# cristicbz/rust-doom

Measured on NVIDIA H100. Metric: frames/sec at 1920x1080 (palette-index bit-exact), higher is better.
Workload: dtype u8

## Files before the change

### rust-doom_b200/csrc/b2d_kernels.cu

```cuda
#include <type_traits>

#include "b2d_kernels.cuh"

namespace b2d {

namespace {

constexpr unsigned kFull = 0xFFFFFFFFu;

constexpr int kMaskWords = 128;
constexpr int kStackDepth = 128;

constexpr uint32_t kVisBit = 1u << 25, kSolidBit = 1u << 24;
__device__ __forceinline__ uint32_t pack_range(int lo, int hi, uint32_t bits) {
    return (uint32_t)lo | ((uint32_t)hi << 12) | bits;
}
__device__ __forceinline__ int range_lo(uint32_t r) { return (int)(r & 0xFFFu); }
__device__ __forceinline__ int range_hi(uint32_t r) { return (int)((r >> 12) & 0xFFFu); }

__device__ __forceinline__ uint32_t word_bits(int w, int lo, int hi) {
    int a = max(lo, w * 32), b = min(hi, w * 32 + 31);
    if (a > b) return 0u;
    uint32_t m = 0xFFFFFFFFu >> (31 - (b - w * 32));
    return m & (0xFFFFFFFFu << (a - w * 32));
// ... 360 lines not shown

constexpr int kBatch = 8;

template <bool kRgba, int kW>
__device__ __forceinline__ void store_batch(const RasterCtx &c, uint8_t *p8, uint32_t *p32, const uint32_t (&v)[kBatch],
                                            int y, int ya, int yb, bool full) {
    const int Wc = kW ? kW : c.W;
    if (full) {
#pragma unroll
        for (int k = 0; k < kBatch; k++) put_px<kRgba>(c, p8 + (size_t)k * Wc, kRgba ? p32 + (size_t)k * Wc : nullptr, true, v[k]);
    } else {
        const uint32_t m = row_mask(y, ya, yb, kBatch);
#pragma unroll
        for (int k = 0; k < kBatch; k++)
            put_px<kRgba>(c, p8 + (size_t)k * Wc, kRgba ? p32 + (size_t)k * Wc : nullptr, (m >> k) & 1u, v[k]);
    }
}

template <bool kRgba, int kW>
__device__ __forceinline__ void fill_void_warp(const RasterCtx &c, int ya, int yb) {
    bool act = ya < yb;
    int y0 = __reduce_min_sync(kFull, act ? ya : 0x7FFFFFFF);
    int y1 = __reduce_max_sync(kFull, act ? yb : 0);
    if (y0 >= y1) return;
    const int Wc = kW ? kW : c.W;
    uint8_t *p8 = c.fb + (size_t)y0 * Wc;
    uint32_t *p32 = kRgba ? c.rgba + (size_t)y0 * Wc : nullptr;
#pragma unroll 1
    for (int y = y0; y < y1; y++, p8 += Wc, p32 += Wc) put_px<kRgba>(c, p8, p32, y >= ya && y < yb, 0u);
}

template <bool kRgba, int kW>
__device__ __forceinline__ void draw_sky_warp(const RasterCtx &c, int ya, int yb) {
    const DeviceScene &sc = *c.sc;
    if (sc.sky_tex < 0) { fill_void_warp<kRgba, kW>(c, ya, yb); return; }
    const TexRec T = sc.tex[sc.sky_tex];
    const bool inter = tex_interleaved(T);
    const uint8_t *px = sc.lit_texels + T.texel_off + (inter ? 4u * c.skycol : c.skycol);
    const uint32_t w4 = 4u * T.w;
    bool act = ya < yb;
    int y0 = __reduce_min_sync(kFull, act ? ya : 0x7FFFFFFF);
    int y1 = __reduce_max_sync(kFull, act ? yb : 0);
    if (y0 >= y1) return;
    const int Wc = kW ? kW : c.W;
    uint8_t *p8 = c.fb + (size_t)y0 * Wc;
    uint32_t *p32 = kRgba ? c.rgba + (size_t)y0 * Wc : nullptr;
#pragma unroll 2
    for (int y = y0; y < y1; y++, p8 += Wc, p32 += Wc) {
        const uint32_t r = sc.skyrow[y];
        put_px<kRgba>(c, p8, p32, y >= ya && y < yb, __ldg(px + (inter ? (r >> 2) * w4 + (r & 3u) : r * T.w)));
    }
}

template <bool kRgba, int kW, bool kFixed = false>
__device__ __forceinline__ void draw_plane_warp(const RasterCtx &c, const FrameConst &fc, const View &vw,
                                                int ya, int yb, int32_t h, int32_t flat, int lightb,
                                                bool visible) {
    const DeviceScene &sc = *c.sc;
    if (!__any_sync(kFull, ya < yb)) return;
    if (!visible) { fill_void_warp<kRgba, kW>(c, ya, yb); return; }
    if (flat == kFlatSky) { draw_sky_warp<kRgba, kW>(c, ya, yb); return; }
    if (flat < 0 || flat >= sc.nflats) { fill_void_warp<kRgba, kW>(c, ya, yb); return; }
    const uint8_t *lit_flats = sc.lit_flats;
    int fixed_row = -1;
    if constexpr (kFixed) {
        lit_flats = c.fix.row == 32 ? c.fix.flats : lit_flats;
        fixed_row = c.fix.row == 32 ? 0 : c.fix.row;
    }
    const uint64_t px_hi = reinterpret_cast<uint64_t>(lit_flats) & 0xFFFFFFFF00000000ull;
    const uint32_t habs = plane_habs(h, fc.pose.z);
    bool act = ya < yb;
    int y0 = __reduce_min_sync(kFull, act ? ya : 0x7FFFFFFF);
    int y1 = __reduce_max_sync(kFull, act ? yb : 0);
    const int full_lo = __reduce_max_sync(kFull, act ? ya : 0x7FFFFFFF);
    const int full_hi = __reduce_min_sync(kFull, act ? yb : 0);
    const int Wc = kW ? kW : c.W;
    uint8_t *p8 = c.fb + (size_t)y0 * Wc;
    uint32_t *p32 = kRgba ? c.rgba + (size_t)y0 * Wc : nullptr;
    const uint32_t bu = (uint32_t)fc.pose.x << 10, bv = (uint32_t)fc.pose.y << 10;
    const uint32_t ax = (uint32_t)c.dir.ax, ay = (uint32_t)c.dir.ay;
    for (int yc = y0; yc < y1; yc += 32) {
        int yy = yc + c.lane;
        if (yy < y1) {
            const PlaneRow pr = plane_row(habs, sc.yslope[yy]);
            c.rowz[c.lane] = make_uint2(pr.z8q, (sc.lit_flat_stride >> 6) * (uint32_t)(kFixed && fixed_row >= 0 ? fixed_row : light_row(lightb, pr.z8)) + 64u * (uint32_t)flat);
        }
        __syncwarp();
        const int rows = min(32, y1 - yc);
        int j = 0;
        for (; j + kBatch <= rows; j += kBatch, p8 += (size_t)kBatch * Wc, p32 += (size_t)kBatch * Wc) {
            uint32_t v[kBatch];
#pragma unroll
            for (int k = 0; k < kBatch; k++) {
                const uint2 rz = c.rowz[j + k];
                v[k] = __ldg(reinterpret_cast<const uint8_t *>(px_hi | flat_offset(rz.y, bu + rz.x * ax, bv + rz.x * ay)));
            }
            const int y = yc + j;
            store_batch<kRgba, kW>(c, p8, p32, v, y, ya, yb, y >= full_lo && y + kBatch <= full_hi);
        }
        for (; j < rows; j++, p8 += Wc, p32 += Wc) {
            const uint2 rz = c.rowz[j];
            const int y = yc + j;
            put_px<kRgba>(c, p8, p32, y >= ya && y < yb,
                          __ldg(reinterpret_cast<const uint8_t *>(px_hi | flat_offset(rz.y, bu + rz.x * ax, bv + rz.x * ay))));
        }
        __syncwarp();
    }
}

template <bool kRgba, int kW, int R>
__device__ __forceinline__ void wall_fast_loop(const RasterCtx &c, const uint8_t *plq, uint32_t w4, uint32_t nq, uint32_t q,
                                               uint32_t acc, uint32_t ts29, int y0, int y1, int ya, int yb,
                                               int full_lo, int full_hi) {
    const int Wc = kW ? kW : c.W;
    uint8_t *p8 = c.fb + (size_t)y0 * Wc;
    uint32_t *p32 = kRgba ? c.rgba + (size_t)y0 * Wc : nullptr;
    asm("" : "+l"(plq));
#pragma unroll 1
    for (int y = y0; y < y1; y += R, p8 += (size_t)R * Wc, p32 += (size_t)R * Wc) {
        const uint32_t q1 = q + 1u == nq ? 0u : q + 1u;
        const uint32_t w0 = __ldg(reinterpret_cast<const uint32_t *>(plq + (size_t)q * w4));
        const uint32_t w1 = __ldg(reinterpret_cast<const uint32_t *>(plq + (size_t)q1 * w4));
        if (y >= full_lo && y + R <= full_hi) {
#pragma unroll
            for (int k = 0; k < R; k++) {
                uint32_t v = pick_byte(w0, w1, wall_sel(acc, ts29, (uint32_t)k));
                if (kRgba) v &= 0xFFu;
                put_px<kRgba>(c, p8 + (size_t)k * Wc, kRgba ? p32 + (size_t)k * Wc : nullptr, true, v);
            }
        } else {
            const uint32_t m = row_mask(y, ya, yb, R);
#pragma unroll
            for (int k = 0; k < R; k++) {
                uint32_t v = pick_byte(w0, w1, wall_sel(acc, ts29, (uint32_t)k));
                if (kRgba) v &= 0xFFu;
                put_px<kRgba>(c, p8 + (size_t)k * Wc, kRgba ? p32 + (size_t)k * Wc : nullptr, (m >> k) & 1u, v);
            }
        }
        wall_advance(acc, q, ts29, (uint32_t)R, nq);
    }
}

template <bool kRgba, int kW, bool kFixed = false>
__device__ __forceinline__ void draw_wall_warp(const RasterCtx &c, const FrameConst &fc, int ya, int yb,
                                               int32_t tex, int32_t tA, int32_t hA, int32_t ucol,
                                               int32_t iscale, int row) {
    const DeviceScene &sc = *c.sc;
    if (!__any_sync(kFull, ya < yb)) return;
    if (tex < 0 || tex >= sc.ntex) { fill_void_warp<kRgba, kW>(c, ya, yb); return; }
    const TexRec T = sc.tex[tex];
    bool act = ya < yb;
    const uint32_t col = (uint32_t)floormod32(ucol, (int32_t)T.w);
    const uint8_t *pl = sc.lit_texels + (size_t)row * sc.lit_texel_stride + T.texel_off;
    if constexpr (kFixed) {
        if (row == 32) pl = c.fix.texels + T.texel_off;
    }
    const uint32_t tstep = (uint32_t)(iscale >> 4);
    int y0 = __reduce_min_sync(kFull, act ? ya : 0x7FFFFFFF);
    int y1 = __reduce_max_sync(kFull, act ? yb : 0);
    const int full_lo = __reduce_max_sync(kFull, act ? ya : 0x7FFFFFFF);
    const int full_hi = __reduce_min_sync(kFull, act ? yb : 0);
    uint32_t t = (uint32_t)wall_tbase(tA, hA, fc.pose.z, c.H, iscale) + (uint32_t)y0 * tstep;
    const int Wc = kW ? kW : c.W;
    uint8_t *p8 = c.fb + (size_t)y0 * Wc;
    uint32_t *p32 = kRgba ? c.rgba + (size_t)y0 * Wc : nullptr;
    if (tex_interleaved(T) && T.h >= 8u) {
        const uint32_t ts = act ? tstep : 0u;
        const bool f16 = __all_sync(kFull, ts <= kWallFast16);
        if (f16 || __all_sync(kFull, ts <= kWallFast8)) {
            const uint32_t tt = act ? t : 0u;
            const uint32_t r0 = wall_row((int32_t)tt, T.h, T.hmagic, T.hbias);
            const uint8_t *plq = pl + 4u * col;
            if (f16) wall_fast_loop<kRgba, kW, 16>(c, plq, 4u * T.w, T.h >> 2, r0 >> 2, wall_acc29(tt, r0), ts << 13, y0, y1, ya, yb, full_lo, full_hi);
            else wall_fast_loop<kRgba, kW, 8>(c, plq, 4u * T.w, T.h >> 2, r0 >> 2, wall_acc29(tt, r0), ts << 13, y0, y1, ya, yb, full_lo, full_hi);
            return;
        }
    }
    if (tex_interleaved(T)) {
        const uint32_t colb = 4u * col, w4 = 4u * T.w;
        for (int y = y0; y < y1; y += kBatch, p8 += (size_t)kBatch * Wc, p32 += (size_t)kBatch * Wc, t += (uint32_t)kBatch * tstep) {
            const uint32_t r0 = wall_row((int32_t)t, T.h, T.hmagic, T.hbias);
            const uint32_t acc = wall_acc(t, r0);
            const uint32_t b7 = (acc + 7u * tstep) >> 16;
            uint32_t v[kBatch];
            if (__all_sync(kFull, b7 < 8u)) {
                const uint32_t q0 = r0 >> 2, q1 = next_quad(q0, T.h);
                const uint32_t w0 = __ldg(reinterpret_cast<const uint32_t *>(pl + (q0 * w4 + colb)));
                const uint32_t w1 = __ldg(reinterpret_cast<const uint32_t *>(pl + (q1 * w4 + colb)));
#pragma unroll
                for (int k = 0; k < kBatch; k++) {
                    v[k] = pick_byte(w0, w1, (acc + (uint32_t)k * tstep) >> 16);
                    if (kRgba) v[k] &= 0xFFu;
                }
            } else {
                const uint32_t t4 = t + 4u * tstep;
                const uint32_t r4 = wall_row((int32_t)t4, T.h, T.hmagic, T.hbias);
                const uint32_t acc4 = wall_acc(t4, r4);
                if (__all_sync(kFull, ((acc + 3u * tstep) >> 16) < 8u && ((acc4 + 3u * tstep) >> 16) < 8u)) {
                    const uint32_t q0 = r0 >> 2, q4 = r4 >> 2;
                    const uint32_t a0 = __ldg(reinterpret_cast<const uint32_t *>(pl + (q0 * w4 + colb)));
                    const uint32_t a1 = __ldg(reinterpret_cast<const uint32_t *>(pl + (next_quad(q0, T.h) * w4 + colb)));
                    const uint32_t b0 = __ldg(reinterpret_cast<const uint32_t *>(pl + (q4 * w4 + colb)));
                    const uint32_t b1 = __ldg(reinterpret_cast<const uint32_t *>(pl + (next_quad(q4, T.h) * w4 + colb)));
#pragma unroll
                    for (int k = 0; k < 4; k++) {
                        v[k] = pick_byte(a0, a1, (acc + (uint32_t)k * tstep) >> 16);
                        v[k + 4] = pick_byte(b0, b1, (acc4 + (uint32_t)k * tstep) >> 16);
                        if (kRgba) { v[k] &= 0xFFu; v[k + 4] &= 0xFFu; }
                    }
                } else {
#pragma unroll
                    for (int k = 0; k < kBatch; k++) {
                        const uint32_t rk = wall_row((int32_t)(t + (uint32_t)k * tstep), T.h, T.hmagic, T.hbias);
                        v[k] = __ldg(pl + ((rk >> 2) * w4 + colb + (rk & 3u)));
                    }
                }
            }
            store_batch<kRgba, kW>(c, p8, p32, v, y, ya, yb, y >= full_lo && y + kBatch <= full_hi);
        }
    } else {
        const uint8_t *px = pl + col;
#pragma unroll 1
        for (int y = y0; y < y1; y++, p8 += Wc, p32 += Wc, t += tstep)
            put_px<kRgba>(c, p8, p32, y >= ya && y < yb, __ldg(px + wall_row((int32_t)t, T.h, T.hmagic, T.hbias) * T.w));
    }
}

__device__ __forceinline__ uint32_t *masked_entry(const DeviceScene &sc, const uint32_t *chunks, int e) {
    return sc.masked_list + ((size_t)chunks[e / kMaskedChunk] * kMaskedChunk + (size_t)(e % kMaskedChunk)) * 33u;
}
__device__ __forceinline__ uint32_t *masked_push(const DeviceScene &sc, uint32_t *chunks, int &mcount, int lane) {
    bool ok = mcount < sc.masked_cap;
    if (ok && mcount % kMaskedChunk == 0) {
        uint32_t id = 0;
        if (lane == 0) id = atomicAdd(sc.masked_counter, 1u);
        id = __shfl_sync(kFull, id, 0);
        ok = id < sc.masked_chunks;
        if (ok && lane == 0) chunks[mcount / kMaskedChunk] = id;
        __syncwarp();
    }
    if (!ok) {
        if (lane == 0) atomicOr(sc.status_flag, kStatusMaskedFull);
        return nullptr;
    }
    return masked_entry(sc, chunks, mcount++);
}

template <bool kRgba, int kW, bool kStates, bool kLevels, typename... Fix>
__device__ __noinline__ void masked_pass(const DeviceScene &sc, const View &vw, int32_t pose_z, uint8_t *fb,
                                         uint32_t *rgba, uint32_t pal_s, int x, int lane,
                                         const SegFrame *wl, const uint32_t *chunks, int count, Fix... fix) {
    constexpr bool kFixed = sizeof...(Fix) != 0;
    static_assert(sizeof...(Fix) == 0 || sizeof...(Fix) == 2, "the fixed colormap: the row-32 texel plane and the row");
    struct { const uint8_t *texels; int row; } const fw{fix...};
    RasterCtx c;
    c.sc = &sc; c.pal_s = pal_s; c.fb = fb; c.rgba = rgba;
    c.W = vw.W; c.H = vw.H; c.x = x; c.lane = lane;
    const int Wc = kW ? kW : c.W;
    for (int e = count - 1; e >= 0; e--) {
        const uint32_t *ml = masked_entry(sc, chunks, e);
        const uint32_t k = ml[0];
        const uint32_t packed = ml[1 + c.lane];
        int ya = (int)(packed & 0xFFFFu), yb = (int)(packed >> 16);
        const SegFrame sf = wl[k];
        int32_t tex, tA, hA, ucol = 0, iscale = 1, row = 0;
        if (is_sprite_entry(sf)) {
            SpriteFrame sp;
            const SpriteRec P = sc.sprites[entry_sprite(sf, sp)];
            if (P.tex < 0 || P.tex >= sc.ntex) continue;
            const int32_t sw = (int32_t)sc.tex[P.tex].w, sh = (int32_t)sc.tex[P.tex].h;
            const int64_t scale = sprite_scale(vw, sp.cz);
            int32_t z8;
            scale_depth(vw, scale, iscale, z8);
            row = kFixed && fw.row >= 0 ? fw.row : light_row_sprite(P.light, z8);
            tex = P.tex; tA = 0; hA = P.low + sh;
            if (ya < yb) {
                clip_rows(P.low + sh, P.low, row_scale(scale), pose_z, c.H, ya, yb);
// ... 31 lines not shown
        const uint32_t tstep = (uint32_t)(iscale >> 4);
        uint32_t t = (uint32_t)wall_tbase(tA, hA, pose_z, c.H, iscale) + (uint32_t)y0 * tstep;
        uint8_t *p8 = c.fb + (size_t)y0 * Wc;
        uint32_t *p32 = kRgba ? c.rgba + (size_t)y0 * Wc : nullptr;
        const uint32_t len = act ? (uint32_t)(yb - ya) : 0u;
        if (inter) {
            const uint32_t colb = 4u * col, w4 = 4u * T.w;
#pragma unroll 1
            for (int y = y0; y < y1; y += kBatch, p8 += (size_t)kBatch * Wc, p32 += (size_t)kBatch * Wc, t += (uint32_t)kBatch * tstep) {
                const uint32_t r0 = wall_row((int32_t)t, T.h, T.hmagic, T.hbias);
                const uint32_t acc = wall_acc(t, r0);
                const uint32_t d = (uint32_t)(y - ya);
                uint32_t v[kBatch], o[kBatch];
                if (__all_sync(kFull, ((acc + 7u * tstep) >> 16) < 8u)) {
                    const uint32_t o0 = (r0 >> 2) * w4 + colb, o1 = next_quad(r0 >> 2, T.h) * w4 + colb;
                    const uint32_t w0 = __ldg(reinterpret_cast<const uint32_t *>(pl + o0));
                    const uint32_t w1 = __ldg(reinterpret_cast<const uint32_t *>(pl + o1));
                    uint32_t m0 = 0x01010101u, m1 = 0x01010101u;
                    if (has_mask) {
                        m0 = __ldg(reinterpret_cast<const uint32_t *>(pm + o0));
                        m1 = __ldg(reinterpret_cast<const uint32_t *>(pm + o1));
                    }
#pragma unroll
                    for (int k = 0; k < kBatch; k++) {
                        const uint32_t bk = (acc + (uint32_t)k * tstep) >> 16;
                        v[k] = pick_byte(w0, w1, bk) & 0xFFu;
                        o[k] = pick_byte(m0, m1, bk) & 0xFFu;
                    }
                } else {
#pragma unroll
                    for (int k = 0; k < kBatch; k++) {
                        const uint32_t rk = wall_row((int32_t)(t + (uint32_t)k * tstep), T.h, T.hmagic, T.hbias);
                        const uint32_t off = (rk >> 2) * w4 + colb + (rk & 3u);
                        v[k] = __ldg(pl + off);
                        o[k] = has_mask ? (uint32_t)__ldg(pm + off) : 1u;
                    }
                }
#pragma unroll
                for (int k = 0; k < kBatch; k++)
                    put_px<kRgba>(c, p8 + (size_t)k * Wc, kRgba ? p32 + (size_t)k * Wc : nullptr, d + (uint32_t)k < len && o[k] != 0u, v[k]);
            }
        } else {
#pragma unroll 1
            for (int y = y0; y < y1; y++, p8 += Wc, p32 += Wc, t += tstep) {
                const uint32_t off = wall_row((int32_t)t, T.h, T.hmagic, T.hbias) * T.w + col;
                const bool on = (uint32_t)(y - ya) < len && (!has_mask || __ldg(pm + off) != 0);
                put_px<kRgba>(c, p8, p32, on, __ldg(pl + off));
            }
        }
    }
}

constexpr int kRasterWarps = 8;

constexpr uint32_t kQueueWords = 6144;
constexpr uint32_t kQueueRecs = kQueueWords / 32;
constexpr uint32_t kRecWall = 1u << 16, kRecVisible = 1u << 17;

constexpr int kBandRows = 256;
constexpr int kMaxBands = (2160 + kBandRows - 1) / kBandRows;
constexpr uint32_t kItemCap = 1024;
static_assert(kBandRows % 32 == 0 && kMaxBands <= 256 && kQueueRecs <= 256, "an item is record | band << 8 in 16 bits");

struct DrawQueue {
    uint4 *head;
    uint32_t *ext;
    uint32_t *pool;
    uint32_t *nrec, *nwords;
};

__device__ __forceinline__ bool queue_push(const DrawQueue &q, int lane, uint32_t meta, int32_t a, int32_t b, int32_t c,
                                           int ya, int yb, int32_t ucol, uint32_t iscale_row) {
    const bool act = ya < yb;
    if (!__any_sync(kFull, act)) return true;
    const uint32_t y0 = __reduce_min_sync(kFull, act ? (uint32_t)ya : 0xFFFFu);
    const uint32_t y1 = __reduce_max_sync(kFull, act ? (uint32_t)yb : 0u);
    const bool wall = meta & kRecWall;
    const uint32_t words = wall ? 96u : 32u;
    uint32_t off = 0, i = kQueueRecs;
    if (lane == 0) {
        off = atomicAdd(q.nwords, words);
        if (off + words <= kQueueWords) i = atomicAdd(q.nrec, 1u);
    }
    i = __shfl_sync(kFull, i, 0);
    if (i >= kQueueRecs) return false;
    off = __shfl_sync(kFull, off, 0);
    q.pool[off + lane] = act ? (uint32_t)ya | ((uint32_t)yb << 16) : 0u;
    if (wall) {
        q.pool[off + 32 + lane] = (uint32_t)ucol;
        q.pool[off + 64 + lane] = iscale_row;
    }
    if (lane == 0) {
        q.head[i] = make_uint4(meta | off, (uint32_t)a, (uint32_t)b, (uint32_t)c);
        q.ext[i] = y0 | y1 << 16;
    }
    return true;
}

template <typename T, typename A, typename... P>
__device__ __forceinline__ const T &extra_tables(const A &a, const P &...p) {
    if constexpr (std::is_same_v<T, A>) return a;
    else return extra_tables<T>(p...);
}

template <bool kRgba, int kW, bool kMasked, bool kStates, bool kLevels, typename... Extra>
__global__ void __launch_bounds__(32 * kRasterWarps, 16 / kRasterWarps)
b2d_raster_kernel(const __grid_constant__ DeviceScene sc, const __grid_constant__ View vw, const FrameConst *__restrict__ frames,
                  const SegFrame *__restrict__ work, int stride, int n, int strips,
                  uint8_t *__restrict__ index_fb, uint32_t *__restrict__ rgba_fb, const __grid_constant__ LevelTables lt,
                  const Extra... fx) {
    constexpr bool kFixed = (std::is_same_v<Extra, FixedTables> || ...);
    constexpr bool kSeen = (std::is_same_v<Extra, SeenTables> || ...);
    static_assert(sizeof...(Extra) == (int)kFixed + (int)kSeen, "appended tables: FixedTables, SeenTables, each at most once");
    static_assert(!kFixed || (kStates && kLevels), "fixed colormaps come with per-frame levels and states");
    static_assert(!kSeen || !kRgba, "the seen variant draws index frames only");
    __shared__ uint32_t s_pal[kRgba ? (kLevels ? 256 * kRasterWarps : 256) : 1];
    __shared__ uint2 s_rowz[kRasterWarps][32];
    __shared__ uint32_t s_chunks[kRasterWarps][kMasked ? kMaskedCapMax / kMaskedChunk : 1];
    __shared__ int4 s_lanes[kRasterWarps][32];
    __shared__ int s_frame[kRasterWarps];
    __shared__ uint4 s_qhead[kQueueRecs];
    __shared__ uint32_t s_qext[kQueueRecs];
    __shared__ uint32_t s_qpool[kQueueWords];
    __shared__ uint16_t s_items[kItemCap];
    __shared__ uint32_t s_band[kMaxBands];
    __shared__ uint32_t s_qn[5];
    __shared__ DeviceScene s_scn[kStates || kLevels ? kRasterWarps : 1];
    __shared__ FixedWarp s_fix[kFixed ? kRasterWarps : 1];
    if (threadIdx.x < 5) s_qn[threadIdx.x] = 0;
    for (int b = threadIdx.x; b < kMaxBands; b += blockDim.x) s_band[b] = 0;
    if (kRgba && !kLevels) {
        for (int i = threadIdx.x; i < 256; i += blockDim.x) s_pal[i] = sc.palette[i];
    }
    __syncthreads();

    const int lane = threadIdx.x & 31, warp = threadIdx.x >> 5;
    const long long gw = (long long)blockIdx.x * (blockDim.x >> 5) + warp;
    const bool has_strip = gw < (long long)n * strips;
    const int frame = has_strip ? (int)(gw / strips) : 0, strip = has_strip ? (int)(gw % strips) : 0;
    const int W = kW ? kW : vw.W, H = vw.H;
    const int x0 = strip * 32, x = x0 + lane;
    const bool inside = has_strip && x < W;
    const DrawQueue q{s_qhead, s_qext, s_qpool, &s_qn[0], &s_qn[1]};

    FrameConst fc{};
    if (has_strip) fc = frames[frame];
    const DeviceScene *scp = &sc;
    if constexpr (kStates || kLevels) {
        DeviceScene *d = &s_scn[warp];
        if (has_strip) {
            const DeviceScene *lsrc = kLevels ? lt.scenes + (uint32_t)fc.level : &sc;
            const uint32_t *src = reinterpret_cast<const uint32_t *>(lsrc);
            uint32_t *dst = reinterpret_cast<uint32_t *>(d);
            for (int i = lane; i < (int)(sizeof(DeviceScene) / 4); i += 32) dst[i] = src[i];
            if (kLevels && kRgba) {
                const uint32_t *pal = lsrc->palette;
                for (int i = lane; i < 256; i += 32) s_pal[256 * warp + i] = pal[i];
            }
            __syncwarp();
            if constexpr (kStates) {
                if (lane == 0) {
                    const TableSet t = lt.sets[(uint32_t)fc.set];
                    d->tex = t.tex; d->sectors = t.sectors; d->segs = t.segs; d->sprites = t.sprites; d->mids = t.mids;
                }
                __syncwarp();
            }
        }
        scp = d;
    }
    if constexpr (kFixed) {
        if (has_strip && lane == 0) {
            const FixedTables &t = extra_tables<FixedTables>(fx...);
            const FixedPlanes p = t.planes[(uint32_t)fc.level];
            s_fix[warp] = FixedWarp{p.texels, p.flats, t.frame_fixed[frame]};
        }
        __syncwarp();
    }
    const DeviceScene &ts = *scp;
    const DeviceScene &ls = kLevels ? ts : sc;
    RasterCtx c;
    c.sc = &ts;
    if constexpr (kFixed) c.fix = s_fix[warp];
    c.pal_s = (uint32_t)__cvta_generic_to_shared(kLevels ? s_pal + 256 * warp : s_pal);
    c.rowz = s_rowz[warp];
    c.W = W; c.H = H; c.x = x; c.lane = lane;
    int mcount = 0;
    uint32_t *chunks = s_chunks[warp];
    asm("" : "+l"(chunks));
    const SegFrame *wl = work + (size_t)frame * stride;

    if (has_strip) {
    c.dir = plane_dir(fc, vw, inside ? x : 0, ls.invF);
    c.fb = index_fb + (size_t)frame * W * H + (inside ? x : 0);
    c.rgba = kRgba ? rgba_fb + (size_t)frame * W * H + (inside ? x : 0) : nullptr;
    c.skycol = 0;
    if (ls.sky_tex >= 0 && inside) c.skycol = umulhi32(sky_u32(x, vw, fc.pose.angle), ts.tex[ls.sky_tex].w);
    s_lanes[warp][lane] = make_int4(c.dir.ax, c.dir.ay, (int)c.skycol, inside ? x : 0);
    if (lane == 0) s_frame[warp] = frame;

    int ct = 0, cb = inside ? H : 0;
    const bool defer = kMasked && ls.masked_list != nullptr;
    const int count = fc.count;
    const uint32_t owner = (uint32_t)warp << 18;
    bool done = false;
    uint32_t *seen_row = nullptr;
    const int32_t *seen_line = nullptr;
    int32_t seen_last = -1;
    if constexpr (kSeen) {
        const SeenTables &st = extra_tables<SeenTables>(fx...);
        seen_row = st.rows + (size_t)frame * st.words;
        seen_line = st.seg_line + st.level_off[kLevels ? (uint32_t)fc.level : 0u];
    }

    for (int k0 = 0; k0 < count && !done; k0 += 32) {
        int k = k0 + lane;
        bool overlap = false;
        if (k < count) {
            int xlo = wl[k].xlo, xhi = wl[k].xhi;
            overlap = xhi >= x0 && xlo <= x0 + 31;
        }
        unsigned m = __ballot_sync(kFull, overlap);
        while (m) {
            int j = __ffs(m) - 1;
            m &= m - 1;
            if (!__any_sync(kFull, ct < cb)) { done = true; break; }
            const SegFrame sf = wl[k0 + j];
            bool in = inside && ct < cb && x >= sf.xlo && x <= sf.xhi;
            if (!__any_sync(kFull, in)) continue;
            if (is_sprite_entry(sf)) {
                if (defer) {
                    uint32_t *ml = masked_push(ls, chunks, mcount, lane);
                    if (ml) {
                        if (lane == 0) ml[0] = (uint32_t)(k0 + j);
                        ml[1 + lane] = in ? ((uint32_t)ct | ((uint32_t)cb << 16)) : 0u;
                    }
                }
                continue;
            }
            ColumnEval ce = {0u, 1, 1, 0};
            bool ok = in && column_eval(sf, vw, x, ce);
            if (!__any_sync(kFull, ok)) continue;
            if constexpr (kSeen) {
                if (lane == 0) {
                    const int32_t l = __ldg(seen_line + sf.seg);
                    if (l >= 0 && l != seen_last) {
                        atomicOr(seen_row + (l >> 5), 1u << (l & 31));
                        seen_last = l;
                    }
                }
            }

            const SegRec S = ts.segs[sf.seg];
            const SectorRec SF = ts.sectors[S.front];
            const int32_t fcl = SF.ceil, ffl = SF.floor;
            const bool two = S.flags & kSegTwoSided;
            const bool ceil_vis = plane_visible(true, fcl, SF.ceil_flat == kFlatSky, fc.pose.z);
            const bool floor_vis = plane_visible(false, ffl, SF.floor_flat == kFlatSky, fc.pose.z);

            WallRows wr = {ct, ct, ct, ct};
            int yend = ct, row = 0;
            int32_t ucol = 0;
            if (ok) {
                row = kFixed && c.fix.row >= 0 ? c.fix.row : light_row(S.light, ce.z8);
                ucol = wall_column(S.uoff, S.len_q12, ce.s24);
                wr = wall_rows(fcl, ffl, two, S.otop, S.obot, ce.scale, fc.pose.z, H, ct, cb);
                yend = cb;
            }
#pragma unroll 1
            for (int pz = 0; pz < 2; pz++) {
                const bool top = pz == 0;
                const int ya = ok ? (top ? ct : wr.y4) : 0, yb = ok ? (top ? wr.y1 : yend) : 0;
                const int32_t h = top ? fcl : ffl, flat = top ? SF.ceil_flat : SF.floor_flat;
                const bool vis = top ? ceil_vis : floor_vis;
                if (!queue_push(q, lane, owner | (vis ? kRecVisible : 0u), h, flat, SF.light, ya, yb, 0, 0u))
                    draw_plane_warp<kRgba, kW, kFixed>(c, fc, vw, ya, yb, h, flat, SF.light, vis);
            }
#pragma unroll 1
            for (int pw = 0; pw < 2; pw++) {
                const bool upper = pw == 0;
                if (!wall_piece(upper, two, fcl, ffl, S.otop, S.obot)) continue;
                const int ya = ok ? (upper ? wr.y1 : wr.y3) : 0, yb = ok ? (upper ? wr.y2 : wr.y4) : 0;
                const int32_t tex = upper ? S.texA : S.texB, tA = upper ? S.tA : S.tB, hA = upper ? S.hA : S.hB;
                if (!queue_push(q, lane, owner | kRecWall, tex, tA, hA, ya, yb, ucol, (uint32_t)ce.iscale | ((uint32_t)row << 24)))
                    draw_wall_warp<kRgba, kW, kFixed>(c, fc, ya, yb, tex, tA, hA, ucol, ce.iscale, row);
            }
            if (ok) wall_window(two, wr, H, ct, cb);
            if (defer && two && S.mid >= 0) {
                const bool keep = ok && wr.y2 < wr.y3;
                if (__any_sync(kFull, keep)) {
                    uint32_t *ml = masked_push(ls, chunks, mcount, lane);
                    if (ml) {
                        if (lane == 0) ml[0] = (uint32_t)(k0 + j);
                        ml[1 + lane] = keep ? ((uint32_t)wr.y2 | ((uint32_t)wr.y3 << 16)) : 0u;
                    }
                }
            }
        }
    }
    if (!queue_push(q, lane, owner, 0, 0, 0, inside ? ct : 0, inside ? cb : 0, 0, 0u))
        fill_void_warp<kRgba, kW>(c, inside ? ct : 0, inside ? cb : 0);
    }

    if (kMasked && mcount > 0 && lane == 0) s_qn[4] = 1;
    __syncthreads();
    const uint32_t nrec = min(s_qn[0], kQueueRecs);
    for (uint32_t r = threadIdx.x; r < nrec; r += blockDim.x) {
        const uint32_t e = s_qext[r];
        for (uint32_t b = (e & 0xFFFFu) / kBandRows; b <= ((e >> 16) - 1u) / kBandRows; b++) atomicAdd(&s_band[b], 1u);
    }
    __syncthreads();
    if (warp == 0) {
        constexpr int kPer = (kMaxBands + 31) / 32;
        uint32_t v[kPer], sum = 0;
#pragma unroll
        for (int k = 0; k < kPer; k++) {
            const int b = lane * kPer + k;
            v[k] = b < kMaxBands ? s_band[b] : 0u;
            sum += v[k];
        }
        uint32_t incl = sum;
#pragma unroll
        for (int d = 1; d < 32; d <<= 1) {
            const uint32_t u = __shfl_up_sync(kFull, incl, d);
            if (lane >= d) incl += u;
        }
        uint32_t at = incl - sum;
#pragma unroll
        for (int k = 0; k < kPer; k++) {
            const int b = lane * kPer + k;
            if (b < kMaxBands) s_band[b] = at;
            at += v[k];
        }
        if (lane == 31) s_qn[3] = incl;
    }
    __syncthreads();
    const bool banded = s_qn[3] <= kItemCap && !(kMasked && s_qn[4]);
    if (banded) {
        for (uint32_t r = threadIdx.x; r < nrec; r += blockDim.x) {
            const uint32_t e = s_qext[r];
            for (uint32_t b = (e & 0xFFFFu) / kBandRows; b <= ((e >> 16) - 1u) / kBandRows; b++)
                s_items[atomicAdd(&s_band[b], 1u)] = (uint16_t)(r | b << 8);
        }
        __syncthreads();
    }
    const uint32_t nitems = banded ? s_qn[3] : nrec;
    for (;;) {
        uint32_t i = 0;
        if (lane == 0) i = atomicAdd(&s_qn[2], 1u);
        i = __shfl_sync(kFull, i, 0);
        if (i >= nitems) break;
        int lo = 0, hi = H;
        if (banded) {
            const uint32_t it = s_items[i];
            i = it & 0xFFu;
            lo = (int)(it >> 8) * kBandRows;
            hi = lo + kBandRows;
        }
        const uint4 hd = s_qhead[i];
        const uint32_t off = hd.x & 0xFFFFu, o = hd.x >> 18;
        const int4 ln = s_lanes[o][lane];
        const int f = s_frame[o];
        const FrameConst fo = frames[f];
        RasterCtx d;
        d.sc = kStates || kLevels ? &s_scn[o] : &sc;
        if constexpr (kFixed) d.fix = s_fix[o];
        d.pal_s = (uint32_t)__cvta_generic_to_shared(kLevels ? s_pal + 256 * o : s_pal);
        d.rowz = s_rowz[warp];
        d.dir = PlaneDir{ln.x, ln.y};
        d.fb = index_fb + (size_t)f * W * H + ln.w;
        d.rgba = kRgba ? rgba_fb + (size_t)f * W * H + ln.w : nullptr;
        d.W = W; d.H = H; d.x = ln.w; d.lane = lane;
        d.skycol = (uint32_t)ln.z;
        const uint32_t win = s_qpool[off + lane];
        const int ya = max((int)(win & 0xFFFFu), lo), yb = min((int)(win >> 16), hi);
        if (hd.x & kRecWall) {
            const uint32_t isr = s_qpool[off + 64 + lane];
            draw_wall_warp<kRgba, kW, kFixed>(d, fo, ya, yb, (int32_t)hd.y, (int32_t)hd.z, (int32_t)hd.w, (int32_t)s_qpool[off + 32 + lane],
                                      (int32_t)(isr & 0xFFFFFFu), (int)(isr >> 24));
        } else {
            draw_plane_warp<kRgba, kW, kFixed>(d, fo, vw, ya, yb, (int32_t)hd.y, (int32_t)hd.z, (int)hd.w, hd.x & kRecVisible);
        }
    }
    if constexpr (kMasked) {
        __syncthreads();
        if constexpr (kFixed) {
            if (mcount > 0) masked_pass<kRgba, kW, kStates, kLevels>(ts, vw, fc.pose.z, c.fb, c.rgba, c.pal_s, x, lane, wl, chunks, mcount, c.fix.texels, c.fix.row);
        } else {
            if (mcount > 0) masked_pass<kRgba, kW, kStates, kLevels>(ts, vw, fc.pose.z, c.fb, c.rgba, c.pal_s, x, lane, wl, chunks, mcount);
        }
    }
}

__global__ void __launch_bounds__(256)
b2d_palette_kernel(const uint32_t *__restrict__ palette, const uint8_t *__restrict__ index,
                   uint32_t *__restrict__ rgba, size_t n_pixels) {
    __shared__ uint32_t s_pal[256];
    s_pal[threadIdx.x] = palette[threadIdx.x];
    __syncthreads();
    const bool aligned = ((reinterpret_cast<uintptr_t>(index) | reinterpret_cast<uintptr_t>(rgba)) & 15) == 0;
    const size_t nvec = aligned ? n_pixels / 16 : 0;
    const size_t stride = (size_t)gridDim.x * blockDim.x;
    for (size_t i = (size_t)blockIdx.x * blockDim.x + threadIdx.x; i < nvec; i += stride) {
        uint4 in = __ldcs(reinterpret_cast<const uint4 *>(index) + i);
        uint32_t wds[4] = {in.x, in.y, in.z, in.w};
        uint4 *out = reinterpret_cast<uint4 *>(rgba) + 4 * i;
#pragma unroll
        for (int q = 0; q < 4; q++) {
            uint4 o;
            o.x = s_pal[wds[q] & 0xFF];
            o.y = s_pal[(wds[q] >> 8) & 0xFF];
            o.z = s_pal[(wds[q] >> 16) & 0xFF];
            o.w = s_pal[wds[q] >> 24];
            __stcs(out + q, o);
        }
    }
    for (size_t p = nvec * 16 + (size_t)blockIdx.x * blockDim.x + threadIdx.x; p < n_pixels; p += stride)
        rgba[p] = s_pal[index[p]];
}

__global__ void __launch_bounds__(256)
b2d_palette_levels_kernel(const uint32_t *__restrict__ palettes, const uint32_t *__restrict__ tables,
                          const uint8_t *__restrict__ index, uint32_t *__restrict__ rgba, size_t npix, int parts) {
    __shared__ uint32_t s_pal[256];
    const size_t frame = blockIdx.x / parts;
    const int part = blockIdx.x % parts;
    s_pal[threadIdx.x] = palettes[(size_t)tables[frame] * 256 + threadIdx.x];
    __syncthreads();
    const uint8_t *in = index + frame * npix;
    uint32_t *out = rgba + frame * npix;
    const bool aligned = npix % 16 == 0 && ((reinterpret_cast<uintptr_t>(index) | reinterpret_cast<uintptr_t>(rgba)) & 15) == 0;
    const size_t n = aligned ? npix / 16 : npix;
    const size_t per = (n + parts - 1) / parts, lo = (size_t)part * per, hi = lo + per < n ? lo + per : n;
    if (aligned) {
// ... 590 lines not shown
```

### rust-doom_b200/csrc/b2d_math.cuh

```cuda
#pragma once
#include <stdint.h>

#if defined(__CUDACC__)
#define B2D_HD __host__ __device__ __forceinline__
#else
#define B2D_HD inline
#endif

namespace b2d {

struct Pose { int32_t x, y, z; uint32_t angle; };
struct View { int32_t W, H, F, FY2; };

struct FrameConst {
    Pose pose;
    int32_t cosq, sinq;
    int32_t px8, py8;
    int32_t count;
    int32_t status;
    int32_t set;
    int32_t level;
    int32_t pad[4];
};
static_assert(sizeof(FrameConst) == 64, "FrameConst");
// ... 243 lines not shown
    if (r2 == 0) r2 = 1;
    const uint64_t s = ((uint64_t)vw.FY2 << 16) / (uint32_t)r2;
    return s > 0xFFFFFFFFull ? 0xFFFFFFFFu : (uint32_t)s;
}

B2D_HD uint32_t plane_habs(int32_t h, int32_t pose_z) {
    int64_t hrel = clampv<int64_t>(((int64_t)h << 16) - pose_z, -((int64_t)1 << 27), (int64_t)1 << 27);
    return (uint32_t)(hrel < 0 ? -hrel : hrel);
}
B2D_HD int32_t wall_hrel(int32_t h, int32_t pose_z) {
    return (int32_t)clampv<int64_t>(((int64_t)h << 16) - pose_z, -((int64_t)1 << 27), (int64_t)1 << 27);
}

struct PlaneDir { int32_t ax, ay; };
B2D_HD PlaneDir plane_dir(const FrameConst &f, const View &vw, int x, uint32_t invF) {
    const int64_t c2 = 2 * (int64_t)x + 1 - vw.W;
    const int64_t nx = ((int64_t)f.cosq * vw.F + (int64_t)f.sinq * c2) >> 4;
    const int64_t ny = ((int64_t)f.sinq * vw.F - (int64_t)f.cosq * c2) >> 4;
    const int64_t m = (int64_t)invF << 24;
    PlaneDir d;
#if defined(__CUDA_ARCH__)
    d.ax = (int32_t)__mul64hi(nx, m);
    d.ay = (int32_t)__mul64hi(ny, m);
#else
    d.ax = (int32_t)(int64_t)(((__int128)nx * m) >> 64);
    d.ay = (int32_t)(int64_t)(((__int128)ny * m) >> 64);
#endif
    return d;
}
struct PlaneRow { uint32_t z8q; int32_t z8; };
B2D_HD PlaneRow plane_row(uint32_t habs, uint32_t yslope) {
    PlaneRow pr;
    uint64_t zz = ((uint64_t)habs * yslope) >> 16;
    int32_t z16 = zz > 0x7FFFFFFFull ? 0x7FFFFFFF : (int32_t)zz;
    pr.z8q = (uint32_t)(z16 >> 8);
    int32_t z8 = z16 >> 13;
    pr.z8 = z8 > 65535 ? 65535 : z8;
    return pr;
}
B2D_HD uint32_t plane_u(int32_t pose_xy, uint32_t z8q, int32_t a) { return ((uint32_t)pose_xy << 10) + z8q * (uint32_t)a; }
B2D_HD uint32_t flat_index(uint32_t U, uint32_t V) { return ((U >> 26) << 6) | (V >> 26); }
B2D_HD uint32_t flat_offset(uint32_t cm6, uint32_t U, uint32_t V) {
#if defined(__CUDA_ARCH__)
    return __funnelshift_l(V, cm6 + (U >> 26), 6);
#else
    return ((cm6 + (U >> 26)) << 6) | (V >> 26);
#endif
}

B2D_HD int32_t wall_tbase(int32_t tA, int32_t hA, int32_t pose_z, int32_t H, int32_t iscale) {
    int64_t t = ((int64_t)tA << 16) + wall_hrel(hA, pose_z) + (((int64_t)(1 - H) * iscale) >> 5);
    return (int32_t)t;
}
B2D_HD uint32_t wall_row(int32_t t, uint32_t h, uint32_t hmagic, uint32_t hbias) {
    uint32_t n = ((uint32_t)t + (hbias << 16)) >> 16;
    uint32_t q = umulhi32(n, hmagic);
    const uint32_t r = n - q * h;
    return r < h ? r : 0u;
}

B2D_HD bool tex_interleaved(uint32_t h, uint32_t texel_off) { return (h & 3u) == 0u && (texel_off & 3u) == 0u && h <= 4096u; }
B2D_HD uint32_t lit_index(bool inter, uint32_t w, uint32_t row, uint32_t col) {
    return inter ? ((row >> 2) * w + col) * 4u + (row & 3u) : row * w + col;
}
B2D_HD uint32_t wall_acc(uint32_t t, uint32_t r0) { return (t & 0xFFFFu) | ((r0 & 3u) << 16); }
B2D_HD uint32_t next_quad(uint32_t q0, uint32_t h) { return q0 + 1u == (h >> 2) ? 0u : q0 + 1u; }
B2D_HD uint32_t pick_byte(uint32_t lo, uint32_t hi, uint32_t sel) {
#if defined(__CUDA_ARCH__)
    uint32_t d;
    asm("prmt.b32 %0, %1, %2, %3;" : "=r"(d) : "r"(lo), "r"(hi), "r"(sel));
    return d;
#else
    return ((sel & 4u) ? hi : lo) >> (8u * (sel & 3u)) & 0xFFu;
#endif
}

constexpr uint32_t kWallFast8 = 32768u;
constexpr uint32_t kWallFast16 = 16384u;
B2D_HD uint32_t wall_acc29(uint32_t t, uint32_t r0) { return ((r0 & 3u) << 29) | ((t & 0xFFFFu) << 13); }
B2D_HD uint32_t wall_sel(uint32_t acc, uint32_t ts29, uint32_t k) { return (acc + k * ts29) >> 29; }
B2D_HD void wall_advance(uint32_t &acc, uint32_t &q, uint32_t ts29, uint32_t R, uint32_t nq) {
    acc += R * ts29;
    q += acc >> 31;
    if (q >= nq) q -= nq;
    acc &= 0x7FFFFFFFu;
}
B2D_HD uint32_t row_mask(int y, int ya, int yb, int R) {
    int lo = ya - y, hi = yb - y;
    if (lo < 0) lo = 0;
    if (hi > R) hi = R;
    if (hi <= lo) return 0u;
    return ((1u << hi) - 1u) & ~((1u << lo) - 1u);
}

B2D_HD uint32_t sky_u32(int x, const View &vw, uint32_t angle) {
    uint64_t num = ((uint64_t)(2 * x + 1)) << 32;
    return (uint32_t)(num / (uint32_t)vw.W) - (angle << 3);
}
B2D_HD int32_t sky_row(int y, int32_t H, int32_t skyh) {
    int32_t r = 2 * y + 1;
    if (r < H) return (r * skyh) / H;
    return floormod32(((2 * H - r) * skyh) / H, skyh);
}

constexpr int32_t kBoxNearQ8 = 32 * 256;
B2D_HD bool box_range(const FrameConst &f, const View &vw, const int32_t box[4], int &lo, int &hi) {
// ... 229 lines not shown
```

Baseline: 616,000.

## Precompute wall/plane record headers at enqueue time and halve band rows

Wall and plane draw records now carry precomputed headers: texture column offset, loop path selection, fused t-key with hbias folded in, hmagic and dims for walls; habs, flat and light for planes. The raster consumer no longer re-reads TexRec, FrameConst or recomputes the path ballots per band. Pose-derived bu/bv now live in a per-warp owner slot in shared memory. The band height drops from 256 to 128 rows, which should improve balance across warps but adds more items and more per-item overhead.

```diff
diff --git a/rust-doom_b200/csrc/b2d_kernels.cu b/rust-doom_b200/csrc/b2d_kernels.cu
--- a/rust-doom_b200/csrc/b2d_kernels.cu
+++ b/rust-doom_b200/csrc/b2d_kernels.cu
@@ -436,15 +436,24 @@
     }
 }
 
+constexpr uint32_t kRecWall = 1u << 16, kRecVisible = 1u << 17, kRecSky = 1u << 21;
+constexpr int kRecPathShift = 22;
+constexpr uint32_t kLoopPlain = 0, kLoopInter = 1, kLoopFast8 = 2, kLoopFast16 = 3;
+
+__device__ __forceinline__ uint4 plane_head(const DeviceScene &sc, bool visible, int32_t h, int32_t flat, int lightb, int32_t pose_z) {
+    if (!visible || (flat != kFlatSky && (flat < 0 || flat >= sc.nflats))) return make_uint4(0u, 0u, 0u, 0u);
+    if (flat == kFlatSky) return make_uint4(kRecVisible | kRecSky, 0u, 0u, 0u);
+    return make_uint4(kRecVisible, plane_habs(h, pose_z), (uint32_t)flat, (uint32_t)lightb);
+}
+
 template <bool kRgba, int kW, bool kFixed = false>
-__device__ __forceinline__ void draw_plane_warp(const RasterCtx &c, const FrameConst &fc, const View &vw,
-                                                int ya, int yb, int32_t h, int32_t flat, int lightb,
-                                                bool visible) {
+__device__ __forceinline__ void draw_plane_warp(const RasterCtx &c, uint32_t bu, uint32_t bv, int ya, int yb, const uint4 &head) {
     const DeviceScene &sc = *c.sc;
     if (!__any_sync(kFull, ya < yb)) return;
-    if (!visible) { fill_void_warp<kRgba, kW>(c, ya, yb); return; }
-    if (flat == kFlatSky) { draw_sky_warp<kRgba, kW>(c, ya, yb); return; }
-    if (flat < 0 || flat >= sc.nflats) { fill_void_warp<kRgba, kW>(c, ya, yb); return; }
+    if (!(head.x & kRecVisible)) { fill_void_warp<kRgba, kW>(c, ya, yb); return; }
+    if (head.x & kRecSky) { draw_sky_warp<kRgba, kW>(c, ya, yb); return; }
+    const uint32_t habs = head.y, flat = head.z;
+    const int lightb = (int)head.w;
     const uint8_t *lit_flats = sc.lit_flats;
     int fixed_row = -1;
     if constexpr (kFixed) {
@@ -452,7 +461,6 @@
         fixed_row = c.fix.row == 32 ? 0 : c.fix.row;
     }
     const uint64_t px_hi = reinterpret_cast<uint64_t>(lit_flats) & 0xFFFFFFFF00000000ull;
-    const uint32_t habs = plane_habs(h, fc.pose.z);
     bool act = ya < yb;
     int y0 = __reduce_min_sync(kFull, act ? ya : 0x7FFFFFFF);
     int y1 = __reduce_max_sync(kFull, act ? yb : 0);
@@ -461,13 +469,12 @@
     const int Wc = kW ? kW : c.W;
     uint8_t *p8 = c.fb + (size_t)y0 * Wc;
     uint32_t *p32 = kRgba ? c.rgba + (size_t)y0 * Wc : nullptr;
-    const uint32_t bu = (uint32_t)fc.pose.x << 10, bv = (uint32_t)fc.pose.y << 10;
     const uint32_t ax = (uint32_t)c.dir.ax, ay = (uint32_t)c.dir.ay;
     for (int yc = y0; yc < y1; yc += 32) {
         int yy = yc + c.lane;
         if (yy < y1) {
             const PlaneRow pr = plane_row(habs, sc.yslope[yy]);
-            c.rowz[c.lane] = make_uint2(pr.z8q, (sc.lit_flat_stride >> 6) * (uint32_t)(kFixed && fixed_row >= 0 ? fixed_row : light_row(lightb, pr.z8)) + 64u * (uint32_t)flat);
+            c.rowz[c.lane] = make_uint2(pr.z8q, (sc.lit_flat_stride >> 6) * (uint32_t)(kFixed && fixed_row >= 0 ? fixed_row : light_row(lightb, pr.z8)) + 64u * flat);
         }
         __syncwarp();
         const int rows = min(32, y1 - yc);
@@ -525,52 +532,56 @@
     }
 }
 
-template <bool kRgba, int kW, bool kFixed = false>
-__device__ __forceinline__ void draw_wall_warp(const RasterCtx &c, const FrameConst &fc, int ya, int yb,
-                                               int32_t tex, int32_t tA, int32_t hA, int32_t ucol,
-                                               int32_t iscale, int row) {
-    const DeviceScene &sc = *c.sc;
+__device__ __forceinline__ uint4 wall_head(const DeviceScene &sc, int32_t tex, int32_t tA, int32_t hA, int32_t pose_z, bool act,
+                                          int32_t ucol, int32_t iscale, int row, bool fixed32, uint32_t &coff) {
+    coff = 0u;
+    if (tex < 0 || tex >= sc.ntex) return make_uint4(0u, 0u, 0u, 0u);
+    const TexRec T = sc.tex[tex];
+    const bool inter = tex_interleaved(T);
+    const uint32_t col = (uint32_t)floormod32(ucol, (int32_t)T.w);
+    coff = (fixed32 ? 0u : (uint32_t)row * sc.lit_texel_stride) + T.texel_off + (inter ? 4u * col : col);
+    uint32_t path = inter ? kLoopInter : kLoopPlain;
+    if (inter && T.h >= 8u) {
+        const uint32_t ts = act ? (uint32_t)(iscale >> 4) : 0u;
+        path = __all_sync(kFull, ts <= kWallFast16) ? kLoopFast16 : __all_sync(kFull, ts <= kWallFast8) ? kLoopFast8 : path;
+    }
+    return make_uint4(kRecWall | path << kRecPathShift, wall_tkey(tA, hA, pose_z, T.hbias), T.hmagic, T.w | T.h << 16);
+}
+
+template <bool kRgba, int kW>
+__device__ __forceinline__ void draw_wall_warp(const RasterCtx &c, const uint8_t *planes, const uint4 &head, int ya, int yb,
+                                               uint32_t coff, int32_t iscale) {
     if (!__any_sync(kFull, ya < yb)) return;
-    if (tex < 0 || tex >= sc.ntex) { fill_void_warp<kRgba, kW>(c, ya, yb); return; }
-    const TexRec T = sc.tex[tex];
+    const uint32_t path = (head.x >> kRecPathShift) & 3u, hmagic = head.z, tw = head.w & 0xFFFFu, th = head.w >> 16;
+    const uint8_t *pl = planes + coff;
     bool act = ya < yb;
-    const uint32_t col = (uint32_t)floormod32(ucol, (int32_t)T.w);
-    const uint8_t *pl = sc.lit_texels + (size_t)row * sc.lit_texel_stride + T.texel_off;
-    if constexpr (kFixed) {
-        if (row == 32) pl = c.fix.texels + T.texel_off;
-    }
     const uint32_t tstep = (uint32_t)(iscale >> 4);
     int y0 = __reduce_min_sync(kFull, act ? ya : 0x7FFFFFFF);
     int y1 = __reduce_max_sync(kFull, act ? yb : 0);
     const int full_lo = __reduce_max_sync(kFull, act ? ya : 0x7FFFFFFF);
     const int full_hi = __reduce_min_sync(kFull, act ? yb : 0);
-    uint32_t t = (uint32_t)wall_tbase(tA, hA, fc.pose.z, c.H, iscale) + (uint32_t)y0 * tstep;
+    uint32_t t = head.y + wall_tcol(c.H, iscale) + (uint32_t)y0 * tstep;
     const int Wc = kW ? kW : c.W;
     uint8_t *p8 = c.fb + (size_t)y0 * Wc;
     uint32_t *p32 = kRgba ? c.rgba + (size_t)y0 * Wc : nullptr;
-    if (tex_interleaved(T) && T.h >= 8u) {
-        const uint32_t ts = act ? tstep : 0u;
-        const bool f16 = __all_sync(kFull, ts <= kWallFast16);
-        if (f16 || __all_sync(kFull, ts <= kWallFast8)) {
-            const uint32_t tt = act ? t : 0u;
-            const uint32_t r0 = wall_row((int32_t)tt, T.h, T.hmagic, T.hbias);
-            const uint8_t *plq = pl + 4u * col;
-            if (f16) wall_fast_loop<kRgba, kW, 16>(c, plq, 4u * T.w, T.h >> 2, r0 >> 2, wall_acc29(tt, r0), ts << 13, y0, y1, ya, yb, full_lo, full_hi);
-            else wall_fast_loop<kRgba, kW, 8>(c, plq, 4u * T.w, T.h >> 2, r0 >> 2, wall_acc29(tt, r0), ts << 13, y0, y1, ya, yb, full_lo, full_hi);
-            return;
-        }
-    }
-    if (tex_interleaved(T)) {
-        const uint32_t colb = 4u * col, w4 = 4u * T.w;
+    if (path >= kLoopFast8) {
+        const uint32_t ts = act ? tstep : 0u, tt = act ? t : 0u;
+        const uint32_t r0 = wall_row((int32_t)tt, th, hmagic, 0u);
+        if (path == kLoopFast16) wall_fast_loop<kRgba, kW, 16>(c, pl, 4u * tw, th >> 2, r0 >> 2, wall_acc29(tt, r0), ts << 13, y0, y1, ya, yb, full_lo, full_hi);
+        else wall_fast_loop<kRgba, kW, 8>(c, pl, 4u * tw, th >> 2, r0 >> 2, wall_acc29(tt, r0), ts << 13, y0, y1, ya, yb, full_lo, full_hi);
+        return;
+    }
+    if (path == kLoopInter) {
+        const uint32_t w4 = 4u * tw;
         for (int y = y0; y < y1; y += kBatch, p8 += (size_t)kBatch * Wc, p32 += (size_t)kBatch * Wc, t += (uint32_t)kBatch * tstep) {
-            const uint32_t r0 = wall_row((int32_t)t, T.h, T.hmagic, T.hbias);
+            const uint32_t r0 = wall_row((int32_t)t, th, hmagic, 0u);
             const uint32_t acc = wall_acc(t, r0);
             const uint32_t b7 = (acc + 7u * tstep) >> 16;
             uint32_t v[kBatch];
             if (__all_sync(kFull, b7 < 8u)) {
-                const uint32_t q0 = r0 >> 2, q1 = next_quad(q0, T.h);
-                const uint32_t w0 = __ldg(reinterpret_cast<const uint32_t *>(pl + (q0 * w4 + colb)));
-                const uint32_t w1 = __ldg(reinterpret_cast<const uint32_t *>(pl + (q1 * w4 + colb)));
+                const uint32_t q0 = r0 >> 2, q1 = next_quad(q0, th);
+                const uint32_t w0 = __ldg(reinterpret_cast<const uint32_t *>(pl + q0 * w4));
+                const uint32_t w1 = __ldg(reinterpret_cast<const uint32_t *>(pl + q1 * w4));
 #pragma unroll
                 for (int k = 0; k < kBatch; k++) {
                     v[k] = pick_byte(w0, w1, (acc + (uint32_t)k * tstep) >> 16);
@@ -578,14 +589,14 @@
                 }
             } else {
                 const uint32_t t4 = t + 4u * tstep;
-                const uint32_t r4 = wall_row((int32_t)t4, T.h, T.hmagic, T.hbias);
+                const uint32_t r4 = wall_row((int32_t)t4, th, hmagic, 0u);
                 const uint32_t acc4 = wall_acc(t4, r4);
                 if (__all_sync(kFull, ((acc + 3u * tstep) >> 16) < 8u && ((acc4 + 3u * tstep) >> 16) < 8u)) {
                     const uint32_t q0 = r0 >> 2, q4 = r4 >> 2;
-                    const uint32_t a0 = __ldg(reinterpret_cast<const uint32_t *>(pl + (q0 * w4 + colb)));
-                    const uint32_t a1 = __ldg(reinterpret_cast<const uint32_t *>(pl + (next_quad(q0, T.h) * w4 + colb)));
-                    const uint32_t b0 = __ldg(reinterpret_cast<const uint32_t *>(pl + (q4 * w4 + colb)));
-                    const uint32_t b1 = __ldg(reinterpret_cast<const uint32_t *>(pl + (next_quad(q4, T.h) * w4 + colb)));
+                    const uint32_t a0 = __ldg(reinterpret_cast<const uint32_t *>(pl + q0 * w4));
+                    const uint32_t a1 = __ldg(reinterpret_cast<const uint32_t *>(pl + next_quad(q0, th) * w4));
+                    const uint32_t b0 = __ldg(reinterpret_cast<const uint32_t *>(pl + q4 * w4));
+                    const uint32_t b1 = __ldg(reinterpret_cast<const uint32_t *>(pl + next_quad(q4, th) * w4));
 #pragma unroll
                     for (int k = 0; k < 4; k++) {
                         v[k] = pick_byte(a0, a1, (acc + (uint32_t)k * tstep) >> 16);
@@ -595,18 +606,17 @@
                 } else {
 #pragma unroll
                     for (int k = 0; k < kBatch; k++) {
-                        const uint32_t rk = wall_row((int32_t)(t + (uint32_t)k * tstep), T.h, T.hmagic, T.hbias);
-                        v[k] = __ldg(pl + ((rk >> 2) * w4 + colb + (rk & 3u)));
+                        const uint32_t rk = wall_row((int32_t)(t + (uint32_t)k * tstep), th, hmagic, 0u);
+                        v[k] = __ldg(pl + ((rk >> 2) * w4 + (rk & 3u)));
                     }
                 }
             }
             store_batch<kRgba, kW>(c, p8, p32, v, y, ya, yb, y >= full_lo && y + kBatch <= full_hi);
         }
     } else {
-        const uint8_t *px = pl + col;
 #pragma unroll 1
         for (int y = y0; y < y1; y++, p8 += Wc, p32 += Wc, t += tstep)
-            put_px<kRgba>(c, p8, p32, y >= ya && y < yb, __ldg(px + wall_row((int32_t)t, T.h, T.hmagic, T.hbias) * T.w));
+            put_px<kRgba>(c, p8, p32, y >= ya && y < yb, __ldg(pl + wall_row((int32_t)t, th, hmagic, 0u) * tw));
     }
 }
 
@@ -744,12 +754,12 @@
 }
 
 constexpr int kRasterWarps = 8;
+static_assert(kRasterWarps <= 8, "a record's owner warp takes the three bits 18-20 of its meta word");
 
 constexpr uint32_t kQueueWords = 6144;
 constexpr uint32_t kQueueRecs = kQueueWords / 32;
-constexpr uint32_t kRecWall = 1u << 16, kRecVisible = 1u << 17;
-
-constexpr int kBandRows = 256;
+
+constexpr int kBandRows = 128;
 constexpr int kMaxBands = (2160 + kBandRows - 1) / kBandRows;
 constexpr uint32_t kItemCap = 1024;
 static_assert(kBandRows % 32 == 0 && kMaxBands <= 256 && kQueueRecs <= 256, "an item is record | band << 8 in 16 bits");
@@ -761,13 +771,12 @@
     uint32_t *nrec, *nwords;
 };
 
-__device__ __forceinline__ bool queue_push(const DrawQueue &q, int lane, uint32_t meta, int32_t a, int32_t b, int32_t c,
-                                           int ya, int yb, int32_t ucol, uint32_t iscale_row) {
+__device__ __forceinline__ bool queue_push(const DrawQueue &q, int lane, const uint4 &head, int ya, int yb, uint32_t w1, uint32_t w2) {
     const bool act = ya < yb;
     if (!__any_sync(kFull, act)) return true;
     const uint32_t y0 = __reduce_min_sync(kFull, act ? (uint32_t)ya : 0xFFFFu);
     const uint32_t y1 = __reduce_max_sync(kFull, act ? (uint32_t)yb : 0u);
-    const bool wall = meta & kRecWall;
+    const bool wall = head.x & kRecWall;
     const uint32_t words = wall ? 96u : 32u;
     uint32_t off = 0, i = kQueueRecs;
     if (lane == 0) {
@@ -779,11 +788,11 @@
     off = __shfl_sync(kFull, off, 0);
     q.pool[off + lane] = act ? (uint32_t)ya | ((uint32_t)yb << 16) : 0u;
     if (wall) {
-        q.pool[off + 32 + lane] = (uint32_t)ucol;
-        q.pool[off + 64 + lane] = iscale_row;
+        q.pool[off + 32 + lane] = w1;
+        q.pool[off + 64 + lane] = w2;
     }
     if (lane == 0) {
-        q.head[i] = make_uint4(meta | off, (uint32_t)a, (uint32_t)b, (uint32_t)c);
+        q.head[i] = make_uint4(head.x | off, head.y, head.z, head.w);
         q.ext[i] = y0 | y1 << 16;
     }
     return true;
@@ -810,7 +819,7 @@
     __shared__ uint2 s_rowz[kRasterWarps][32];
     __shared__ uint32_t s_chunks[kRasterWarps][kMasked ? kMaskedCapMax / kMaskedChunk : 1];
     __shared__ int4 s_lanes[kRasterWarps][32];
-    __shared__ int s_frame[kRasterWarps];
+    __shared__ uint4 s_owner[kRasterWarps];
     __shared__ uint4 s_qhead[kQueueRecs];
     __shared__ uint32_t s_qext[kQueueRecs];
     __shared__ uint32_t s_qpool[kQueueWords];
@@ -888,7 +897,7 @@
     c.skycol = 0;
     if (ls.sky_tex >= 0 && inside) c.skycol = umulhi32(sky_u32(x, vw, fc.pose.angle), ts.tex[ls.sky_tex].w);
     s_lanes[warp][lane] = make_int4(c.dir.ax, c.dir.ay, (int)c.skycol, inside ? x : 0);
-    if (lane == 0) s_frame[warp] = frame;
+    if (lane == 0) s_owner[warp] = make_uint4((uint32_t)frame, (uint32_t)fc.pose.x << 10, (uint32_t)fc.pose.y << 10, 0u);
 
     int ct = 0, cb = inside ? H : 0;
     const bool defer = kMasked && ls.masked_list != nullptr;
@@ -964,17 +973,25 @@
                 const int ya = ok ? (top ? ct : wr.y4) : 0, yb = ok ? (top ? wr.y1 : yend) : 0;
                 const int32_t h = top ? fcl : ffl, flat = top ? SF.ceil_flat : SF.floor_flat;
                 const bool vis = top ? ceil_vis : floor_vis;
-                if (!queue_push(q, lane, owner | (vis ? kRecVisible : 0u), h, flat, SF.light, ya, yb, 0, 0u))
-                    draw_plane_warp<kRgba, kW, kFixed>(c, fc, vw, ya, yb, h, flat, SF.light, vis);
+                uint4 head = plane_head(ts, vis, h, flat, SF.light, fc.pose.z);
+                head.x |= owner;
+                if (!queue_push(q, lane, head, ya, yb, 0u, 0u))
+                    draw_plane_warp<kRgba, kW, kFixed>(c, (uint32_t)fc.pose.x << 10, (uint32_t)fc.pose.y << 10, ya, yb, head);
             }
 #pragma unroll 1
             for (int pw = 0; pw < 2; pw++) {
                 const bool upper = pw == 0;
                 if (!wall_piece(upper, two, fcl, ffl, S.otop, S.obot)) continue;
                 const int ya = ok ? (upper ? wr.y1 : wr.y3) : 0, yb = ok ? (upper ? wr.y2 : wr.y4) : 0;
+                if (!__any_sync(kFull, ya < yb)) continue;
                 const int32_t tex = upper ? S.texA : S.texB, tA = upper ? S.tA : S.tB, hA = upper ? S.hA : S.hB;
-                if (!queue_push(q, lane, owner | kRecWall, tex, tA, hA, ya, yb, ucol, (uint32_t)ce.iscale | ((uint32_t)row << 24)))
-                    draw_wall_warp<kRgba, kW, kFixed>(c, fc, ya, yb, tex, tA, hA, ucol, ce.iscale, row);
+                uint32_t coff;
+                uint4 head = wall_head(ts, tex, tA, hA, fc.pose.z, ya < yb, ucol, ce.iscale, row, kFixed && c.fix.row == 32, coff);
+                head.x |= owner;
+                if (!queue_push(q, lane, head, ya, yb, coff, (uint32_t)ce.iscale)) {
+                    if (head.x & kRecWall) draw_wall_warp<kRgba, kW>(c, kFixed && c.fix.row == 32 ? c.fix.texels : ts.lit_texels, head, ya, yb, coff, ce.iscale);
+                    else fill_void_warp<kRgba, kW>(c, ya, yb);
+                }
             }
             if (ok) wall_window(two, wr, H, ct, cb);
             if (defer && two && S.mid >= 0) {
@@ -989,7 +1006,7 @@
             }
         }
     }
-    if (!queue_push(q, lane, owner, 0, 0, 0, inside ? ct : 0, inside ? cb : 0, 0, 0u))
+    if (!queue_push(q, lane, make_uint4(owner, 0u, 0u, 0u), inside ? ct : 0, inside ? cb : 0, 0u, 0u))
         fill_void_warp<kRgba, kW>(c, inside ? ct : 0, inside ? cb : 0);
     }
 
@@ -1049,10 +1066,10 @@
             hi = lo + kBandRows;
         }
         const uint4 hd = s_qhead[i];
-        const uint32_t off = hd.x & 0xFFFFu, o = hd.x >> 18;
+        const uint32_t off = hd.x & 0xFFFFu, o = (hd.x >> 18) & (kRasterWarps - 1);
         const int4 ln = s_lanes[o][lane];
-        const int f = s_frame[o];
-        const FrameConst fo = frames[f];
+        const uint4 ow = s_owner[o];
+        const int f = (int)ow.x;
         RasterCtx d;
         d.sc = kStates || kLevels ? &s_scn[o] : &sc;
         if constexpr (kFixed) d.fix = s_fix[o];
@@ -1066,11 +1083,10 @@
         const uint32_t win = s_qpool[off + lane];
         const int ya = max((int)(win & 0xFFFFu), lo), yb = min((int)(win >> 16), hi);
         if (hd.x & kRecWall) {
-            const uint32_t isr = s_qpool[off + 64 + lane];
-            draw_wall_warp<kRgba, kW, kFixed>(d, fo, ya, yb, (int32_t)hd.y, (int32_t)hd.z, (int32_t)hd.w, (int32_t)s_qpool[off + 32 + lane],
-                                      (int32_t)(isr & 0xFFFFFFu), (int)(isr >> 24));
+            draw_wall_warp<kRgba, kW>(d, kFixed && d.fix.row == 32 ? d.fix.texels : d.sc->lit_texels, hd, ya, yb, s_qpool[off + 32 + lane],
+                                      (int32_t)s_qpool[off + 64 + lane]);
         } else {
-            draw_plane_warp<kRgba, kW, kFixed>(d, fo, vw, ya, yb, (int32_t)hd.y, (int32_t)hd.z, (int)hd.w, hd.x & kRecVisible);
+            draw_plane_warp<kRgba, kW, kFixed>(d, ow.y, ow.z, ya, yb, hd);
         }
     }
     if constexpr (kMasked) {
diff --git a/rust-doom_b200/csrc/b2d_math.cuh b/rust-doom_b200/csrc/b2d_math.cuh
--- a/rust-doom_b200/csrc/b2d_math.cuh
+++ b/rust-doom_b200/csrc/b2d_math.cuh
@@ -319,6 +319,10 @@
     int64_t t = ((int64_t)tA << 16) + wall_hrel(hA, pose_z) + (((int64_t)(1 - H) * iscale) >> 5);
     return (int32_t)t;
 }
+B2D_HD uint32_t wall_tkey(int32_t tA, int32_t hA, int32_t pose_z, uint32_t hbias) {
+    return ((uint32_t)tA << 16) + (uint32_t)wall_hrel(hA, pose_z) + (hbias << 16);
+}
+B2D_HD uint32_t wall_tcol(int32_t H, int32_t iscale) { return (uint32_t)(((int64_t)(1 - H) * iscale) >> 5); }
 B2D_HD uint32_t wall_row(int32_t t, uint32_t h, uint32_t hmagic, uint32_t hbias) {
     uint32_t n = ((uint32_t)t + (hbias << 16)) >> 16;
     uint32_t q = umulhi32(n, hmagic);
```

After: 619,900, median of 6. Within noise of the previous version (+0.6%).
